# QwenLM/Qwen3-TTS

Measured on AMD Instinct MI355X. Metric: speech-tokens/sec (+ audio RTF), Qwen3-TTS-12Hz-1.7B batch=8, higher is better.
Workload: dtype bf16; 1 GPU; Qwen3-TTS-12Hz-1.7b dims, seeded random weights, batch=8 per GPU, ragged prompts 36..64 rows, 125 frames (10.0 s) per utterance, sampling T=0.9 top-k=50 rep=1.05; prefill + AR decode (hipGraph=on) + codec decode to 24 kHz (bf16); global_batch=8, frames_per_utterance=125, parallelism=request-shard x1

## Files before the change

qwen3-tts_amd/csrc/gemm_tap.hip:

```cpp
#include <map>
#include <mutex>
#include <type_traits>
#include "common.h"
#include "kernels.h"
#include "tstamp.h"

QTTS_TS_UNIT(tap)

namespace qtts {

typedef __bf16 hw_bf16x2 __attribute__((ext_vector_type(2)));
__device__ __forceinline__ unsigned cvt_pk_bf16(float a, float b) {
    hw_bf16x2 v = {(__bf16)a, (__bf16)b};
    return *reinterpret_cast<unsigned*>(&v);
}

template <bool FAST>
__device__ __forceinline__ float snake1(float v, float ea, float ib) {
    float sn;
    if constexpr (FAST) sn = __builtin_amdgcn_sinf(v * ea * 0.15915494309189535f); else sn = sinf(v * ea);
    return v + ib * (sn * sn);
}

template <int BN, int TM, int TN, bool FAST>
// ... 618 lines not shown
        gd_dma_wait();
        __syncthreads();
        if (s + 1 < nsteps) {
            const int ks2 = (s + 1) / p.taps, tap2 = (s + 1) - ks2 * p.taps;
            dma_w(ks2, tap2, (s + 1) & 1);
            if (ks2 != ks) dma_a(ks2, ks2 & 1);
        }
        const bf16_t* Ab = reinterpret_cast<const bf16_t*>(Abuf + (ks & 1) * a_stride);
        const bf16_t* Wb = reinterpret_cast<const bf16_t*>(Wbuf + (s & 1) * W_BYTES);
        const int sh = p.shift[tap];
#pragma unroll
        for (int kk = 0; kk < BK / 32; ++kk) {
            bf16x8 a[TM], b[TN];
#pragma unroll
            for (int i = 0; i < TM; ++i) {
                a[i] = *reinterpret_cast<const bf16x8*>(&Ab[(wm * 64 + i * 16 + li + halo + sh) * STR + kk * 32 + lq * 8]);
                if (tpos[i] + sh < 0) a[i] = (bf16x8){0, 0, 0, 0, 0, 0, 0, 0};
            }
#pragma unroll
            for (int j = 0; j < TN; ++j)
                b[j] = *reinterpret_cast<const bf16x8*>(&Wb[(wn * (BN / 2) + j * 16 + li) * STR + kk * 32 + lq * 8]);
#pragma unroll
            for (int i = 0; i < TM; ++i)
#pragma unroll
                for (int j = 0; j < TN; ++j)
                    acc[i][j] = __builtin_amdgcn_mfma_f32_16x16x32_bf16(b[j], a[i], acc[i][j], 0, 0, 0);
        }
    }
    tap_epilogue<BN, TM, TN, true>(p, acc, m0, n0, wm, wn, li, lq);
}

template <int BN>
static void launch_dma(const GemmTapParams& p, int halo, hipStream_t st) {
    const int nb = cdiv(p.M, 128) * cdiv(p.N, BN);
    const int a_stride = ((128 + halo) * 144 + 1023) / 1024 * 1024;
    const size_t lds = 2 * (size_t)a_stride + 2 * (size_t)((BN * 144 + 1023) / 1024 * 1024);
    auto kern = gemm_dma_kernel<BN>;
    ensure_dynamic_lds(reinterpret_cast<const void*>(kern), 160 * 1024);
    hipLaunchKernelGGL(kern, dim3(nb), dim3(256), lds, st, p, halo, a_stride);
}

__device__ __forceinline__ void ring_wait_vm(int n) {
#ifndef QTTS_HOST_EMU
    switch (n) {
        case 0: asm volatile("s_waitcnt vmcnt(0)" ::: "memory"); break;
        case 2: asm volatile("s_waitcnt vmcnt(2)" ::: "memory"); break;
        case 4: asm volatile("s_waitcnt vmcnt(4)" ::: "memory"); break;
        case 6: asm volatile("s_waitcnt vmcnt(6)" ::: "memory"); break;
        case 8: asm volatile("s_waitcnt vmcnt(8)" ::: "memory"); break;
        case 10: asm volatile("s_waitcnt vmcnt(10)" ::: "memory"); break;
        case 12: asm volatile("s_waitcnt vmcnt(12)" ::: "memory"); break;
        case 14: asm volatile("s_waitcnt vmcnt(14)" ::: "memory"); break;
        case 16: asm volatile("s_waitcnt vmcnt(16)" ::: "memory"); break;
        case 20: asm volatile("s_waitcnt vmcnt(20)" ::: "memory"); break;
        case 24: asm volatile("s_waitcnt vmcnt(24)" ::: "memory"); break;
        case 28: asm volatile("s_waitcnt vmcnt(28)" ::: "memory"); break;
        default: asm volatile("s_waitcnt vmcnt(0)" ::: "memory"); break;
    }
#else
    (void)n;
#endif
}
__device__ __forceinline__ void ring_barrier() {
#ifndef QTTS_HOST_EMU
    asm volatile("s_waitcnt lgkmcnt(0)" ::: "memory");
    __builtin_amdgcn_s_barrier();
    __builtin_amdgcn_sched_barrier(0);
#else
    __syncthreads();
#endif
}
#ifndef QTTS_RING_SGB_ALT
#define QTTS_RING_SGB_ALT 0
#endif
#define QTTS_RING_SGB (QTTS_RING_SGB_ALT == 0 ? 3 : (QTTS_RING_SGB_ALT == 1 ? 0 : QTTS_RING_SGB_ALT))
__device__ __forceinline__ void ring_sched_fence() {
#ifndef QTTS_HOST_EMU
    __builtin_amdgcn_sched_barrier(0);
#endif
}
template <int N> __device__ __forceinline__ void ring_wait_vm_c() {
#ifndef QTTS_HOST_EMU
    asm volatile("s_waitcnt vmcnt(%0)" ::"n"(N) : "memory");
#endif
}
template <int NST, int AH, bool RING_A, int TAPS = 0, int ABL = 0>
__global__ __launch_bounds__(256, 2) void gemm_ring_kernel(GemmTapParams p, int halo, int nbands ,
                                                                 int ks , f32x4* ks_ws, unsigned* ks_cnt) {
    constexpr int BM = 128, BN = 128, TM = 4, TN = 4;
    constexpr int WT = 8192;
    constexpr int D = NST;
    constexpr int LPS = RING_A ? 4 : 2;
    static_assert(!RING_A || AH == 1, "a plain Linear runs 32-wide slabs");
    extern __shared__ __attribute__((aligned(16))) unsigned char smem_gr[];
    unsigned char* Wbuf = smem_gr;
    unsigned char* Abuf = smem_gr + NST * WT;

    const int tid = threadIdx.x;
    const int lane = tid & 63;
    const int wave = __builtin_amdgcn_readfirstlane(tid >> 6);
    const int wm = wave >> 1, wn = wave & 1;
    const int li = lane & 15, lq = lane >> 4;
    const int n_tiles_n = (p.N + BN - 1) / BN;
    const int nblk = gridDim.x;
    int bid = blockIdx.x;
    {
// ... 394 lines not shown
    tab[{dev, st}] = w;
    return w;
}
static int ring_splits(const GemmTapParams& p, int nst, int ah, int n_cu) {
    const int tiles = cdiv(p.M, 128) * cdiv(p.N, 128);
    const int slabs = p.K / (32 * ah), steps = slabs * p.taps * ah;
    int ks = QTTS_OPT_INT("QTTS_GEMM_RING_KS", 0);
    (void)n_cu;
    if (ks == 0) ks = 1;
    while (ks > 1 && (slabs % ks != 0 || tiles * ks > RING_KS_MAX_PARTS || steps / ks < 2 * nst || p.act == ACT_SWIGLU)) --ks;
    return ks < 1 ? 1 : ks;
}
template <int NST, int AH, bool RING_A, int TAPS = 0, int ABL = 0>
static void launch_ring_t(const GemmTapParams& p, int halo, hipStream_t st) {
    static const int n_cu = [] {
        int dev = 0, n = 0;
        if (hipGetDevice(&dev) != hipSuccess || hipDeviceGetAttribute(&n, hipDeviceAttributeMultiprocessorCount, dev) != hipSuccess || n <= 0) n = 256;
        return n;
    }();
    const int nb = cdiv(p.M, 128) * cdiv(p.N, 128);
    const int nbands = (128 + halo + 15) / 16;
    int ks = ring_splits(p, NST, AH, n_cu);
    RingKsWs w{};
    if (ks > 1) { w = ring_ks_ws(st); if (!w.ws) ks = 1; }
    auto kern = gemm_ring_kernel<NST, AH, RING_A, TAPS, ABL>;
    ensure_dynamic_lds(reinterpret_cast<const void*>(kern), 160 * 1024);
    hipLaunchKernelGGL(kern, dim3(nb * ks), dim3(256), (size_t)ring_lds_bytes(NST, AH, p.taps, halo), st, p, halo, nbands, ks, w.ws, w.cnt);
}
static void launch_ring(const GemmTapParams& p, int halo, hipStream_t st) {
    QTTS_REQUIRE((size_t)p.M * p.lda * 2 < (1ull << 32) && (size_t)p.taps * p.N * p.K * 2 < (1ull << 32), QTTS_ERR_LIMIT, "gemm_ring: an operand of 4 GiB or more");
    int nst = QTTS_OPT_INT("QTTS_GEMM_RING_NST", 0);
    if (nst != 4 && nst != 6 && nst != 8) nst = 4;
    const int unroll = QTTS_OPT_INT("QTTS_GEMM_RING_UNROLL", 1);
    if (p.taps == 1) { if (nst == 8) launch_ring_t<8, 1, true>(p, halo, st); else launch_ring_t<4, 1, true>(p, halo, st); return; }
    while (nst > p.taps * 2) nst -= 2;
    QTTS_REQUIRE(nst >= 4, QTTS_ERR_ARG, "gemm_ring: ring deeper than a slab");
#if defined(QTTS_ABLATE) && !defined(QTTS_HOST_EMU)
    if (const int abl = QTTS_OPT_INT("QTTS_GEMM_RING_ABLATE", 0); abl && p.taps == 7) {
        switch (abl) {
            case 1: launch_ring_t<4, 2, false, 7, 1>(p, halo, st); return;
            case 2: launch_ring_t<4, 2, false, 7, 2>(p, halo, st); return;
            case 3: launch_ring_t<4, 2, false, 7, 3>(p, halo, st); return;
            case 4: launch_ring_t<4, 2, false, 7, 4>(p, halo, st); return;
            case 8: launch_ring_t<4, 2, false, 7, 8>(p, halo, st); return;
            case 7: launch_ring_t<4, 2, false, 7, 7>(p, halo, st); return;
            case 15: launch_ring_t<4, 2, false, 7, 15>(p, halo, st); return;
            default: break;
        }
    }
#endif
    if (unroll && p.taps == 7) { if (nst == 8) launch_ring_t<8, 2, false, 7>(p, halo, st); else launch_ring_t<4, 2, false, 7>(p, halo, st); return; }
    if (unroll && p.taps == 2) { launch_ring_t<4, 2, false, 2>(p, halo, st); return; }
    if (nst == 8) launch_ring_t<8, 2, false>(p, halo, st); else if (nst == 6) launch_ring_t<6, 2, false>(p, halo, st); else launch_ring_t<4, 2, false>(p, halo, st);
}

template <int BM, int BN, bool A16, int BK>
static void launch_wide_k(const GemmTapParams& p, hipStream_t st) {
    const int nb = cdiv(p.M, BM) * cdiv(p.N, BN);
    const size_t lds = (size_t)(BM + BN) * (BK + 8) * 2;
    auto kern = gemm_wide_kernel<BM, BN, A16, BK>;
    ensure_dynamic_lds(reinterpret_cast<const void*>(kern), 160 * 1024);
    hipLaunchKernelGGL(kern, dim3(nb), dim3(256), lds, st, p);
}
struct WideTile { int bm, bn, bk; };
static int g_wide_force = -1;
static WideTile wide_tile(const GemmTapParams& p, bool a16, int bn_max) {
    const int force_env = QTTS_OPT_INT("QTTS_GEMM_WIDE_TILE", 0);
    const int force = g_wide_force >= 0 ? g_wide_force : force_env;
    WideTile best{128, bn_max, 128};
    static const int n_cu = [] {
        int dev = 0, n = 0;
        if (hipGetDevice(&dev) != hipSuccess || hipDeviceGetAttribute(&n, hipDeviceAttributeMultiprocessorCount, dev) != hipSuccess || n <= 0) n = 256;
        return n;
    }();
    double tb = 1e30;
    const double ab = a16 ? 2.0 : 4.0;
    for (int cm : {128, 64, 32})
        for (int cn : {128, 64, 32})
            for (int ck : {128, 256}) {
                if (cn > bn_max || p.N % cn != 0 || p.K % ck != 0) continue;
                if (cm == 32 && (p.M > 128 || ck != 256 || cn > 64)) continue;
                if (cn == 32 && (cm != 32 || p.act == ACT_SWIGLU)) continue;
                if (ck == 256 && cm == 64 && !a16 && cn != 64) continue;
                if (ck == 256 && cm == 128) continue;
                if (force && force != (cm * 1000 + cn) * 1000 + ck) continue;
                const int wgs = cdiv(p.M, cm) * cdiv(p.N, cn), steps = p.K / ck;
                const double sb = ck * (cm * ab + cn * 2.0) * 1e-3;
                const double chain = steps * (0.53 + sb / 65.0);
                const double cu = cdiv(wgs, n_cu) * steps * sb / 80.0;
                const double op = (double)cdiv(p.M, cm) * p.N * p.K * 2.0 / 6e6;
                const double t = std::max(chain, std::max(cu, op)) * (1.0 + 0.01 * (cm * cn < 128 * 128));
                if (t < tb) { tb = t; best = {cm, cn, ck}; }
            }
    return best;
}
template <bool A16>
static void launch_wide(const GemmTapParams& p, int bn_max, hipStream_t st) {
    const WideTile t = wide_tile(p, A16, bn_max);
    if (t.bm == 32) { if (t.bn == 64) launch_wide_k<32, 64, A16, 256>(p, st); else launch_wide_k<32, 32, A16, 256>(p, st); return; }
    if (t.bm == 128) { if (t.bn == 128) launch_wide_k<128, 128, A16, 128>(p, st); else launch_wide_k<128, 64, A16, 128>(p, st); }
    else if (t.bk == 128) { if (t.bn == 128) launch_wide_k<64, 128, A16, 128>(p, st); else launch_wide_k<64, 64, A16, 128>(p, st); }
    else if (t.bn == 128) { if constexpr (A16) launch_wide_k<64, 128, true, 256>(p, st); else launch_wide_k<64, 128, false, 128>(p, st); }
    else launch_wide_k<64, 64, A16, 256>(p, st);
}

template <int BN, bool BF16>
static void launch_t(const GemmTapParams& p, hipStream_t st) {
    const int nb = cdiv(p.M, 128) * cdiv(p.N, BN);
    hipLaunchKernelGGL((gemm_tap_kernel<BN, BF16>), dim3(nb), dim3(256), 0, st, p);
}

void launch_gemm_tap(const GemmTapParams& p_in, bool bf16, hipStream_t st) {
    GemmTapParams p = p_in;
    const int wide_max_tiles = [] { const char* e = QTTS_ENV("QTTS_GEMM_WIDE_MAX"); return e && atoi(e) > 0 ? atoi(e) : 2048; }();
    QTTS_REQUIRE(p.K % 32 == 0, QTTS_ERR_ARG, "gemm_tap: K must be a multiple of 32");
    QTTS_REQUIRE(p.taps >= 1 && p.taps <= 8, QTTS_ERR_ARG, "gemm_tap: 1..8 taps");
    QTTS_REQUIRE(p.M > 0 && p.N > 0, QTTS_ERR_ARG, "gemm_tap: empty problem");
    QTTS_REQUIRE(p.lda % 4 == 0, QTTS_ERR_ARG, "gemm_tap: lda must be a multiple of 4");
    auto al16 = [](const void* q) { return reinterpret_cast<uintptr_t>(q) % 16 == 0; };
    p.vec4 = p.N % 4 == 0 && p.ldc % 4 == 0 && (!p.res || p.ldr % 4 == 0) && (!p.C16 || (p.ldc16 % 4 == 0 && reinterpret_cast<uintptr_t>(p.C16) % 8 == 0)) &&
             (!p.res16 || (p.ldres16 % 4 == 0 && reinterpret_cast<uintptr_t>(p.res16) % 8 == 0)) &&
             (!p.R16 || (p.ldR16 % 4 == 0 && reinterpret_cast<uintptr_t>(p.R16) % 8 == 0)) &&
             al16(p.C) && al16(p.res) && al16(p.bias) && al16(p.scale) && al16(p.snake_ea) && al16(p.snake_ib) && al16(p.snake16_ea) &&
             al16(p.snake16_ib) && (p.snake16_period % 4 == 0);
    if (p.act == ACT_SWIGLU) QTTS_REQUIRE(p.ldc % 4 == 0 && al16(p.C) && (!p.C16 || (p.ldc16 % 4 == 0 && reinterpret_cast<uintptr_t>(p.C16) % 8 == 0)),
                                          QTTS_ERR_ARG, "gemm_tap: swiglu outputs must be 16-byte (fp32) / 8-byte (bf16) aligned with ldc % 4 == 0");
    if (p.A16 && bf16 && p.taps == 1 && p.shift[0] == 0 && p.K % 128 == 0 && p.K >= 512 && p.N % 64 == 0 && p.lda % 8 == 0 && (p.C || p.C16) && !p.res16 &&
        !p.R16 && (cdiv(p.M, 128) * cdiv(p.N, 128) <= wide_max_tiles || p.act == ACT_SWIGLU)) {
        if (p.act == ACT_SWIGLU) QTTS_REQUIRE(p.N % 32 == 0, QTTS_ERR_ARG, "gemm_tap: swiglu needs N % 32 == 0");
        {
            const int dma_env2 = [] { const char* e = QTTS_ENV("QTTS_GEMM_DMA"); return e ? atoi(e) : 0; }();
            const int ring_env = QTTS_OPT_INT("QTTS_GEMM_RING", 1);
            if (dma_env2 == 0 && (ring_env == 2 || (ring_env == 1 && cdiv(p.M, 128) * (p.N / 128) >= 128)) && p.N % 128 == 0 && p.K % 64 == 0) {
                launch_ring(p, 0, st);
                QTTS_CHECK_HIP(hipGetLastError());
                return;
            }
            if ((dma_env2 == 1 || dma_env2 == 2) && p.N % 128 == 0 && p.K % 64 == 0 && cdiv(p.M, 128) * (p.N / 128) >= 128) {
                launch_dma<128>(p, 0, st);
                QTTS_CHECK_HIP(hipGetLastError());
                return;
            }
        }
        launch_wide<true>(p, p.N % 128 == 0 ? 128 : 64, st);
        QTTS_CHECK_HIP(hipGetLastError());
        return;
    }
    if (p.A16) {
        QTTS_REQUIRE(bf16, QTTS_ERR_ARG, "gemm_tap: A16 needs bf16 weights");
        QTTS_REQUIRE(p.act != ACT_SWIGLU, QTTS_ERR_ARG, "gemm_tap: the A16 kernel has no SwiGLU epilogue");
        QTTS_REQUIRE(p.lda % 8 == 0, QTTS_ERR_ARG, "gemm_tap: bf16 A needs lda % 8 == 0");
        QTTS_REQUIRE(p.C || p.C16 || p.R16, QTTS_ERR_ARG, "gemm_tap: no output");
        QTTS_REQUIRE(!(p.res && p.res16), QTTS_ERR_ARG, "gemm_tap: residual given twice");
        int halo = 0;
        for (int i = 0; i < p.taps; ++i) { QTTS_REQUIRE(p.shift[i] <= 0, QTTS_ERR_ARG, "gemm_tap: shift > 0"); halo = std::max(halo, -p.shift[i]); }
        QTTS_REQUIRE(halo <= 56, QTTS_ERR_LIMIT, "gemm_tap: tap reach > 56 rows");
        const int bn2 = (p.N % 128 == 0) ? 128 : (p.N % 96 == 0 ? 96 : (p.N <= 64 ? 64 : 128));
        const int bk_env = QTTS_OPT_INT("QTTS_TAP2_BK", 0);
        static const int n_cu2 = [] {
            int dev = 0, n = 0;
            if (hipGetDevice(&dev) != hipSuccess || hipDeviceGetAttribute(&n, hipDeviceAttributeMultiprocessorCount, dev) != hipSuccess || n <= 0) n = 256;
            return n;
        }();
        const int dma_env = [] { const char* e = QTTS_ENV("QTTS_GEMM_DMA"); return e ? atoi(e) : -1; }();
        const int ring_env = QTTS_OPT_INT("QTTS_GEMM_RING", 1);
        if (dma_env != 0 && bn2 == 128 && p.K % 64 == 0 && (ring_env == 2 || (ring_env == 1 && p.taps > 1))) { launch_ring(p, halo, st); QTTS_CHECK_HIP(hipGetLastError()); return; }
        if (dma_env != 0 && bn2 == 128 && p.K % 64 == 0) { launch_dma<128>(p, halo, st); QTTS_CHECK_HIP(hipGetLastError()); return; }
        const int tiles = cdiv(p.M, 128) * cdiv(p.N, bn2);
        const bool bk64 = p.K % 64 == 0 && bn2 == 128 && (bk_env == 64 || (bk_env == 0 && tiles <= n_cu2));
        if (bk64) launch_tap2<128, 64>(p, halo, st);
        else if (bn2 == 128) launch_tap2<128, 32>(p, halo, st); else if (bn2 == 96) launch_tap2<96, 32>(p, halo, st); else launch_tap2<64, 32>(p, halo, st);
        QTTS_CHECK_HIP(hipGetLastError());
        return;
    }
    QTTS_REQUIRE(p.C || (p.C16 && p.act == ACT_SWIGLU), QTTS_ERR_ARG, "gemm_tap: null output");
    QTTS_REQUIRE(!p.res16 && !p.R16, QTTS_ERR_ARG, "gemm_tap: the bf16 residual stream needs the A16 kernel");
    int bn;
    if (p.act == ACT_SWIGLU) {
        QTTS_REQUIRE(p.N % 32 == 0, QTTS_ERR_ARG, "gemm_tap: swiglu needs N % 32 == 0");
        bn = (p.N % 128 == 0) ? 128 : 64;
    } else if (p.N % 128 == 0) bn = 128;
    else if (p.N % 96 == 0) bn = 96;
    else if (p.N <= 64) bn = 64;
    else bn = 128;
    if (bf16 && p.taps == 1 && p.shift[0] == 0 && p.K % 128 == 0 && p.K >= 512 && (bn == 128 || bn == 64) &&
        cdiv(p.M, 128) * cdiv(p.N, bn) <= wide_max_tiles) {
        launch_wide<false>(p, bn, st);
        QTTS_CHECK_HIP(hipGetLastError());
        return;
    }
    if (bf16) {
        if (bn == 128) launch_t<128, true>(p, st);
        else if (bn == 96) launch_t<96, true>(p, st);
        else launch_t<64, true>(p, st);
    } else {
        if (bn == 128) launch_t<128, false>(p, st);
        else if (bn == 96) launch_t<96, false>(p, st);
        else launch_t<64, false>(p, st);
    }
    QTTS_CHECK_HIP(hipGetLastError());
}

extern "C" __attribute__((visibility("default"))) void qtts_debug_gemm_wide_tile(int32_t code) { g_wide_force = code; }
extern "C" __attribute__((visibility("default")))
void qtts_debug_gemm_wide_choice(int32_t M, int32_t N, int32_t K, int32_t a16, int32_t* bm, int32_t* bn, int32_t* bk) {
    GemmTapParams p{};
    p.M = M; p.N = N; p.K = K; p.taps = 1;
    const WideTile t = wide_tile(p, a16 != 0, N % 128 == 0 ? 128 : 64);
    *bm = t.bm; *bn = t.bn; *bk = t.bk;
}

extern "C" __attribute__((visibility("default")))
int qtts_debug_gemm_tap(int32_t M, int32_t N, int32_t K, int32_t act, int32_t with_res, int32_t a16, int32_t iters, int32_t reps,
                        double* us_per_launch) {
    try {
        QTTS_REQUIRE(us_per_launch && iters > 0 && reps > 0 && M > 0, QTTS_ERR_ARG, "bad argument");
        DevBuf A, W, Cb, R;
        A.alloc((size_t)M * K * 4); W.alloc((size_t)N * K * 2); Cb.alloc((size_t)M * N * 4); R.alloc((size_t)M * N * 4);
        QTTS_CHECK_HIP(hipMemset(A.p, 0x3c, A.bytes)); QTTS_CHECK_HIP(hipMemset(W.p, 0x3c, W.bytes)); QTTS_CHECK_HIP(hipMemset(R.p, 0, R.bytes));
        GemmTapParams p{};
        if (a16) p.A16 = A.p; else p.A = A.as<float>();
        p.lda = K; p.M = M; p.T = M; p.W = W.p; p.N = N; p.K = K; p.taps = 1; p.act = act;
        const int No = act == ACT_SWIGLU ? N / 2 : N;
        if (with_res) { p.res = R.as<float>(); p.ldr = No; }
        p.C = Cb.as<float>(); p.ldc = No;
        hipStream_t st;
        QTTS_CHECK_HIP(hipStreamCreateWithFlags(&st, hipStreamNonBlocking));
        launch_gemm_tap(p, true, st);
        QTTS_CHECK_HIP(hipStreamSynchronize(st));
        hipGraph_t gr; hipGraphExec_t ge;
        QTTS_CHECK_HIP(hipStreamBeginCapture(st, hipStreamCaptureModeThreadLocal));
        for (int i = 0; i < iters; ++i) launch_gemm_tap(p, true, st);
        QTTS_CHECK_HIP(hipStreamEndCapture(st, &gr));
        QTTS_CHECK_HIP(hipGraphInstantiate(&ge, gr, nullptr, nullptr, 0));
        QTTS_CHECK_HIP(hipGraphLaunch(ge, st)); QTTS_CHECK_HIP(hipStreamSynchronize(st));
        hipEvent_t a, b;
        QTTS_CHECK_HIP(hipEventCreate(&a)); QTTS_CHECK_HIP(hipEventCreate(&b));
        float best = 1e30f;
        for (int r = 0; r < reps; ++r) {
            QTTS_CHECK_HIP(hipEventRecord(a, st)); QTTS_CHECK_HIP(hipGraphLaunch(ge, st)); QTTS_CHECK_HIP(hipEventRecord(b, st));
            QTTS_CHECK_HIP(hipStreamSynchronize(st));
            float ms = 0; QTTS_CHECK_HIP(hipEventElapsedTime(&ms, a, b)); best = std::min(best, ms);
        }
        *us_per_launch = 1000.0 * best / iters;
        (void)hipEventDestroy(a); (void)hipEventDestroy(b); (void)hipGraphExecDestroy(ge); (void)hipGraphDestroy(gr); (void)hipStreamDestroy(st);
        return QTTS_OK;
    } catch (const qtts::Error& e) { qtts::set_last_error(e.what()); return e.code; }
    catch (const std::exception& e) { qtts::set_last_error(e.what()); return QTTS_ERR_ARG; }
}

extern "C" __attribute__((visibility("default")))
int qtts_debug_gemm_tap16(const void* A16_host, int32_t lda, int32_t M, int32_t T, const void* W_host, int32_t N, int32_t K, int32_t taps,
                          const int32_t* shift, float* C_host, int32_t iters, int32_t reps, double* us_per_launch) {
    try {
        QTTS_REQUIRE(A16_host && W_host && shift && M > 0 && T > 0 && N > 0 && K > 0 && taps >= 1 && taps <= 8 && lda >= K, QTTS_ERR_ARG, "bad argument");
        DevBuf A, W, Cb;
        A.alloc((size_t)M * lda * 2); W.alloc((size_t)taps * N * K * 2); Cb.alloc((size_t)M * N * 4);
        QTTS_CHECK_HIP(hipMemcpy(A.p, A16_host, A.bytes, hipMemcpyHostToDevice));
        QTTS_CHECK_HIP(hipMemcpy(W.p, W_host, W.bytes, hipMemcpyHostToDevice));
        QTTS_CHECK_HIP(hipMemset(Cb.p, 0xff, Cb.bytes));
        GemmTapParams p{};
        p.A16 = A.p; p.lda = lda; p.M = M; p.T = T; p.W = W.p; p.N = N; p.K = K; p.taps = taps;
// ... 33 lines not shown
```

qwen3-tts_amd/csrc/talker_engine.hip:

```cpp
#include <atomic>
#include <map>
#include <mutex>
#include <algorithm>
#include "common.h"
#include "kernels.h"
#include "glue.h"


using namespace qtts;

namespace {

struct LayerW {
    int fs_o = 16, fs_d = 16;
    DevBuf qkv_p, o_p, gu_p, d_p;
    DevBuf gu_p8;
    DevBuf o_p16;
    DevBuf gu_mlp, d_p16;
    DevBuf qkv_r, o_r, gu_r, d_r;
    bool w8 = false;
    DevBuf qkv_s, o_s, gu_s, gu8_s, d_s;
    DevBuf g1, g2, qn, kn;
};
struct StackDims { int H, I, nh, nkv, hd, qd, kvd; float eps; };
// ... 925 lines not shown
        p.res = res; p.ldr = H;
        if (out16) { p.C16 = C; p.ldc16 = ldc; p.ldc = ldc; } else { p.C = C; p.ldc = ldc; }
        launch_gemm_tap(p, bf16, st);
    };
    for (int l = 0; l < c.num_hidden_layers; ++l) {
        auto& L = tl[l];
        if (a16) launch_rmsnorm16(xs, H, L.g1.as<float>(), td.eps, nb, H, M, H, st);
        else launch_rmsnorm(xs, H, L.g1.as<float>(), td.eps, nb, H, M, H, st);
        gemm(L.qkv_r, W, H, nb, H, qb, W, ACT_NONE, nullptr);
        QkNormRopeParams q{};
        q.qkv = qb; q.ld = W; q.B = nB; q.T = T; q.nh = td.nh; q.nkv = td.nkv; q.hd = td.hd; q.qw = L.qn.as<float>();
        q.kw = L.kn.as<float>(); q.eps = td.eps; q.inv_freq = inv_freq_t.as<float>(); q.n_pad = npad_dev;
        q.kv = kv_t; q.layer = l; q.row_map = row_map; q.slot_base = slot_base;
        launch_qknorm_rope_store(q, st);
        AttnRowsParams a{};
        a.qkv = qb; a.ld = W; a.q_off = 0; a.k_off = td.qd; a.v_off = td.qd + td.kvd; a.B = nB; a.T = T; a.nh = td.nh;
        a.nkv = td.nkv; a.hd = td.hd; a.window = 0; a.n_pad = npad_dev; a.out = ab; a.ldo = td.qd;
        if (a16) a.out16 = ab;
        launch_attn_rows(a, st);
        gemm(L.o_r, H, td.qd, ab, td.qd, xs, H, ACT_NONE, xs);
        if (a16) launch_rmsnorm16(xs, H, L.g2.as<float>(), td.eps, nb, H, M, H, st);
        else launch_rmsnorm(xs, H, L.g2.as<float>(), td.eps, nb, H, M, H, st);
        gemm(L.gu_r, 2 * td.I, H, nb, H, mb, td.I, ACT_SWIGLU, nullptr, a16);
        gemm(L.d_r, H, td.I, mb, td.I, xs, H, ACT_NONE, xs);
    }
}

void qtts_talker::prefill(const float* embeds, int B_, int T, const int32_t* n_pad_host, const float* trailing_dev,
                          int Tt_, const float* tts_pad_dev, hipStream_t st) {
    const auto& c = cfg;
    QTTS_REQUIRE(finalized, QTTS_ERR_STATE, "talker: finalize() first");
    QTTS_REQUIRE(B_ >= 1 && B_ <= c.max_batch, QTTS_ERR_LIMIT, "talker: batch exceeds max_batch");
    QTTS_REQUIRE(T >= 1 && T < c.max_seq, QTTS_ERR_LIMIT, "talker: prompt longer than max_seq");
    QTTS_REQUIRE(Tt_ >= 1, QTTS_ERR_ARG, "talker: trailing_text_hidden must have >= 1 row");
    for (int b = 0; b < B_; ++b) QTTS_REQUIRE(n_pad_host[b] >= 0 && n_pad_host[b] < T, QTTS_ERR_ARG, "talker: n_pad out of range");
    if (pooled()) {
        const int want = cdiv(T, 16);
        if (B_ * want > pool_pages)
            throw Error(QTTS_ERR_LIMIT, "talker: the prompts need " + std::to_string(B_ * want) + " KV pages, the pool has " + std::to_string(pool_pages));
        for (int b = 0; b < c.max_batch; ++b) pool_release(b);
        for (int b = 0; b < B_; ++b) pool_grant(b, want);
        pool_flush(st);
    }
    B = B_; T0 = T; Tt = Tt_;
    const int M = B * T, H = td.H;
    pf_x.ensure((size_t)M * H * 4);
    trailing.ensure((size_t)B * Tt * H * 4); tts_pad.ensure((size_t)H * 4);
    QTTS_CHECK_HIP(hipMemcpyAsync(pf_x.p, embeds, (size_t)M * H * 4, hipMemcpyDeviceToDevice, st));
    QTTS_CHECK_HIP(hipMemcpyAsync(trailing.p, trailing_dev, (size_t)B * Tt * H * 4, hipMemcpyDeviceToDevice, st));
    QTTS_CHECK_HIP(hipMemcpyAsync(tts_pad.p, tts_pad_dev, (size_t)H * 4, hipMemcpyDeviceToDevice, st));
    QTTS_CHECK_HIP(hipMemcpyAsync(n_pad_d.p, n_pad_host, (size_t)B * 4, hipMemcpyHostToDevice, st));
    prefill_stack(B, T, n_pad_d.as<int>(), nullptr, 0, st);
    float* xs = pf_x.as<float>();
    for (int b = 0; b < B; ++b)
        QTTS_CHECK_HIP(hipMemcpyAsync(x.as<float>() + (size_t)b * H, xs + ((size_t)b * T + T - 1) * H, (size_t)H * 4,
                                      hipMemcpyDeviceToDevice, st));
    launch_rmsnorm(x.as<float>(), H, t_norm.as<float>(), td.eps, past_hidden.as<float>(), H, B, H, st);
    int init[6] = {0, -1, T - 1, 0, 0, 0};
    QTTS_CHECK_HIP(hipMemcpyAsync(ss.n_generated, init, sizeof(init), hipMemcpyHostToDevice, st));
    std::vector<int> ones(B, 1);
    QTTS_CHECK_HIP(hipMemcpyAsync(ss.unfinished, ones.data(), (size_t)B * 4, hipMemcpyHostToDevice, st));
    SkinnyParams h{};
    h.x = past_hidden.as<float>(); h.ldx = H; h.M = B; h.Wp = head_p.p; h.N = c.vocab_size; h.K = H;
    h.out = logits.as<float>(); h.ldo = c.vocab_size; h.act = ACT_NONE; h.fs = fs_head;
    launch_skinny(h, bf16, st);
    QTTS_CHECK_HIP(hipStreamSynchronize(st));
    prefilled = true;
}

void qtts_talker::sample_talker(const qtts_sampling& sp, int eos, int min_new, int max_new, hipStream_t st) {
    SampleParams p{};
    p.logits = logits.as<float>(); p.ld = cfg.vocab_size; p.V = cfg.vocab_size; p.B = B;
    p.generated = generated.as<int>(); p.gen_stride = gen_cap; p.n_generated_dev = ss.n_generated;
    p.repetition_penalty = sp.repetition_penalty; p.eos = eos; p.min_new_tokens = min_new;
    p.suppress_mask = suppress.as<unsigned char>();
    p.do_sample = sp.do_sample; p.top_k = sp.top_k; p.top_p = sp.top_p; p.temperature = sp.temperature;
    p.seed = sp.seed; p.seed_dev = seed_d.as<unsigned long long>(); p.stream_id = 0; p.step_dev = ss.n_generated;
    p.tok_out = cur_tok.as<int>(); p.tok_stride = 1; p.unfinished = ss.unfinished; p.generated_out = generated.as<int>();
    p.max_new_tokens = max_new; p.done_in = ss.done;
    if (row_mode) { p.rows = rows_d.as<SampleRow>(); p.rows_sub = 0; p.rows_fast = row_fast_t; }
    if (tf.codes && tf.trace) launch_teacher(teacher_params(), 0, st);
    if (row_mode && row_warp_t) { SampleWarpParams pw{p, warp_d.as<RowWarpers>(), proc_d.as<RowProcessors>()}; launch_sample_warp(pw, st); }
    else launch_sample(p, st);
    launch_sample_finish(ss, B, max_new, st);
    if (tf.codes) launch_teacher(teacher_params(), 1, st);
}

void qtts_talker::frame_step(const qtts_sampling& sp, int eos, int min_new, int max_new, int64_t* codes, float* hidden,
                             int max_frames, hipStream_t st) {
    const auto& c = cfg;
    const int G = c.num_code_groups;
    const int64_t fused_before = cp_attn_o_count, mlp_before = cp_mlp_count, layer_before = cp_layer_count, ks_before = ks_split_count, gq_before = attn_gq_count;
    cur_stack = 1;
    for (int j = 0; j < G - 1; ++j) {
        const int n_new = j == 0 ? 2 : 1, M = n_new * B;
        CpGatherParams gp{};
        gp.pass = j; gp.B = B; gp.H = td.H; gp.past_hidden = past_hidden.as<float>(); gp.talker_emb = emb_talker.as<float>();
        gp.cur_tok = cur_tok.as<int>(); gp.cp_emb = emb_cp.as<float>(); gp.cp_vocab = c.cp_vocab_size;
        gp.sub = sub.as<int>(); gp.sub_stride = G; gp.done = ss.done;
        unsigned short* c16 = bf16 ? cp_x16.as<unsigned short>() : nullptr;
        if (has_proj && j >= 1) {
        } else
        if (has_proj) {
            gp.out = cp_in.as<float>(); gp.out16 = bf16 ? cp_in16.as<unsigned short>() : nullptr;
            if (!skinny_only && j == 0) launch_cp_gather(gp, st);
            SkinnyParams pj{};
            pj.done_flag = ss.done;
            pj.x = cp_in.as<float>(); pj.ldx = td.H; pj.M = M; pj.Wp = proj_p.p; pj.N = cd.H; pj.K = td.H;
            if (bf16) { pj.x = reinterpret_cast<const float*>(cp_in16.as<unsigned short>()); pj.x_bf16 = 1; }
            pj.bias = proj_b.as<float>(); pj.out = cp_x.as<float>(); pj.ldo = cd.H; pj.act = ACT_NONE; pj.fs = fs_proj;
// ... 1047 lines not shown
    if (tokens_dev) {
        const int B = t->B, cap = g.admitting ? g.max_row : g.max_new;
        std::vector<int> h((size_t)B * cap);
        copy_on_stream(h.data(), t->generated.p, h.size() * 4, hipMemcpyDeviceToHost, st);
        std::vector<int64_t> w(h.size(), -1);
        for (int b = 0; b < B; ++b)
            for (int i = 0; i < n_tok - (g.admitting ? g.tab[b].origin : 0) && i < cap; ++i) w[(size_t)b * cap + i] = h[(size_t)b * cap + i];
        copy_on_stream(tokens_dev, w.data(), w.size() * 8, hipMemcpyHostToDevice, st);
    }
    QTTS_API_END
}

int qtts_talker_debug_logits(qtts_talker* t, float* logits_dev, void* stream) {
    QTTS_API_BEGIN
    QTTS_REQUIRE(t && logits_dev, QTTS_ERR_ARG, "null argument");
    QTTS_CHECK_HIP(hipMemcpyAsync(logits_dev, t->logits.p, (size_t)t->B * t->cfg.vocab_size * 4, hipMemcpyDeviceToDevice,
                                  (hipStream_t)stream));
    QTTS_API_END
}
int qtts_talker_debug_kv_table(qtts_talker* t, int32_t row, int32_t* entries_host, void* stream) {
    QTTS_API_BEGIN
    QTTS_REQUIRE(t && entries_host, QTTS_ERR_ARG, "null argument");
    QTTS_REQUIRE(t->finalized, QTTS_ERR_STATE, "debug_kv_table before finalize");
    QTTS_REQUIRE(row >= 0 && row < t->cfg.max_batch, QTTS_ERR_ARG, "debug_kv_table: row " + std::to_string(row) + " is not a row of this engine");
    const int pps = t->kv_t.pages_per_seq;
    copy_on_stream(entries_host, t->ptab_t.as<int>() + (size_t)row * pps, (size_t)pps * 4, hipMemcpyDeviceToHost, (hipStream_t)stream);
    QTTS_API_END
}
int qtts_talker_debug_cp_logits(qtts_talker* t, float* logits_dev, void* stream) {
    QTTS_API_BEGIN
    QTTS_REQUIRE(t && logits_dev, QTTS_ERR_ARG, "null argument");
    const size_t Vc = (size_t)t->cfg.cp_vocab_size;
    for (int j = 0; j < t->cfg.num_code_groups - 1; ++j)
        QTTS_CHECK_HIP(hipMemcpyAsync(logits_dev + (size_t)j * t->B * Vc, t->cp_logits.as<float>() + (size_t)j * 64 * Vc, (size_t)t->B * Vc * 4,
                                      hipMemcpyDeviceToDevice, (hipStream_t)stream));
    QTTS_API_END
}
__global__ void xcc_probe_kernel(int* out) {
#ifndef QTTS_HOST_EMU
    if (threadIdx.x == 0) out[blockIdx.x] = (int)__builtin_amdgcn_s_getreg((31 << 11) | 20) & 0xf;
#else
    if (threadIdx.x == 0) out[blockIdx.x] = blockIdx.x & 7;
#endif
}
int qtts_debug_xcc_map(int32_t grid, int32_t* out_host, void* stream) {
    QTTS_API_BEGIN
    QTTS_REQUIRE(grid >= 1 && grid <= 65536 && out_host, QTTS_ERR_ARG, "xcc_map: grid 1..65536");
    DevBuf d; d.alloc((size_t)grid * 4);
    hipLaunchKernelGGL(xcc_probe_kernel, dim3(grid), dim3(256), 0, (hipStream_t)stream, d.as<int>());
    QTTS_CHECK_HIP(hipStreamSynchronize((hipStream_t)stream));
    QTTS_CHECK_HIP(hipMemcpy(out_host, d.p, (size_t)grid * 4, hipMemcpyDeviceToHost));
    QTTS_API_END
}
int qtts_debug_cp_layer_occupancy(int32_t H, int32_t I, int32_t bf16) {
    try { return qtts::cp_layer_blocks_per_cu(H, I, bf16 != 0); } catch (...) { return -1; }
}
int qtts_talker_get_stats(qtts_talker* t, qtts_talker_stats* out) {
    QTTS_API_BEGIN
    QTTS_REQUIRE(t && out, QTTS_ERR_ARG, "null argument");
    out->frames_run = t->frames_run; out->graph_nodes = t->graph_nodes; out->weight_bytes_per_frame = t->weight_bytes_frame;
    out->gemm_ms_last = t->prof_ms; out->gemm_launches_last = t->prof_launches;
    out->long_graphs = (int32_t)t->graph_long.size(); out->attn_nsplit_last = t->attn_nsplit_active; out->attn_span_last = t->attn_span_active;
    out->cp_fused_per_step = t->cp_fused_slot ? t->cp_fused_per_step : 0;
    out->cp_fused_launches_last = (int64_t)out->cp_fused_per_step * t->frames_run;
    out->cp_fused_giveups = t->cp_fused_giveups; out->cp_fused_capacity = t->fused_capacity; out->cp_fused_active = t->cp_fused_slot ? 1 : 0;
    out->cp_mlp_per_step = t->cp_fused_slot ? t->cp_mlp_per_step : 0;
    out->cp_layer_per_step = t->cp_fused_slot ? t->cp_layer_per_step : 0;
    out->ks_split_per_step = t->ks_split_env ? t->ks_split_per_step : 0; out->attn_gq_per_step = t->attn_gq_per_step;
    out->graph_captures = t->graph_captures; out->row_table_last = t->row_mode ? 1 : 0;
    out->admit_calls = (int32_t)t->admit_calls; out->admitted_rows = (int32_t)t->admitted_rows;
    QTTS_API_END
}
int qtts_talker_get_gemm_profile(qtts_talker* t, qtts_gemm_class* out, int32_t cap, int32_t* n) {
    QTTS_API_BEGIN
    QTTS_REQUIRE(t && n && (out || cap == 0), QTTS_ERR_ARG, "null argument");
    *n = (int32_t)t->prof_classes.size();
    for (int i = 0; i < *n && i < cap; ++i) out[i] = t->prof_classes[i];
    QTTS_API_END
}
__global__ void null_kernel(int* p, int mode) {
    if (mode == 1) { if (*p) return; }
    if (mode == 2) { __shared__ int s[64]; s[threadIdx.x & 63] = threadIdx.x; __syncthreads(); if (threadIdx.x == 0 && s[5] == 12345) *p = 1; }
}
int qtts_debug_null_chain(int32_t grid, int32_t block, int32_t mode, int32_t iters, int32_t reps, double* us) {
    QTTS_API_BEGIN
    DevBuf d; d.alloc(64); QTTS_CHECK_HIP(hipMemset(d.p, 0, 64));
    hipStream_t st; QTTS_CHECK_HIP(hipStreamCreateWithFlags(&st, hipStreamNonBlocking));
    hipGraph_t gr; hipGraphExec_t ge;
    QTTS_CHECK_HIP(hipStreamBeginCapture(st, hipStreamCaptureModeThreadLocal));
    for (int i = 0; i < iters; ++i) hipLaunchKernelGGL(null_kernel, dim3(grid), dim3(block), 0, st, d.as<int>(), mode);
    QTTS_CHECK_HIP(hipStreamEndCapture(st, &gr));
    QTTS_CHECK_HIP(hipGraphInstantiate(&ge, gr, nullptr, nullptr, 0));
    QTTS_CHECK_HIP(hipGraphLaunch(ge, st)); QTTS_CHECK_HIP(hipStreamSynchronize(st));
    hipEvent_t a, b; QTTS_CHECK_HIP(hipEventCreate(&a)); QTTS_CHECK_HIP(hipEventCreate(&b));
    float best = 1e30f;
    for (int r = 0; r < reps; ++r) {
        QTTS_CHECK_HIP(hipEventRecord(a, st)); QTTS_CHECK_HIP(hipGraphLaunch(ge, st)); QTTS_CHECK_HIP(hipEventRecord(b, st));
        QTTS_CHECK_HIP(hipStreamSynchronize(st));
        float ms = 0; QTTS_CHECK_HIP(hipEventElapsedTime(&ms, a, b)); best = std::min(best, ms);
    }
    *us = 1000.0 * best / iters;
    (void)hipEventDestroy(a); (void)hipEventDestroy(b); (void)hipGraphExecDestroy(ge); (void)hipGraphDestroy(gr); (void)hipStreamDestroy(st);
    QTTS_API_END
}

int qtts_debug_skinny_chain(int32_t N, int32_t K, int32_t M, int32_t act, int32_t with_norm, int32_t with_res,
// ... 79 lines not shown
```

Baseline: 48310 speech-tokens/s.

## Add smaller-tile DMA ring GEMM for mid-size prefill linears; fuse last-row gather

Adds a new ring-buffered direct-to-LDS GEMM kernel with 64x64 or 128x64 tiles. A planner selects it for prefill-sized linears (M 129..2048, large N and K) whose 128x128 tile count would not fill the CUs, so the grid covers more compute units. Separately, the per-batch device-to-device copies of the last prefill row are removed by having rmsnorm read strided rows directly. It also adds debug entry points, and the new kernel adds more code paths and relies on hand-tuned waitcnt scheduling.

```diff
diff --git a/qwen3-tts_amd/csrc/gemm_tap.hip b/qwen3-tts_amd/csrc/gemm_tap.hip
--- a/qwen3-tts_amd/csrc/gemm_tap.hip
+++ b/qwen3-tts_amd/csrc/gemm_tap.hip
@@ -694,6 +694,7 @@
         case 12: asm volatile("s_waitcnt vmcnt(12)" ::: "memory"); break;
         case 14: asm volatile("s_waitcnt vmcnt(14)" ::: "memory"); break;
         case 16: asm volatile("s_waitcnt vmcnt(16)" ::: "memory"); break;
+        case 18: asm volatile("s_waitcnt vmcnt(18)" ::: "memory"); break;
         case 20: asm volatile("s_waitcnt vmcnt(20)" ::: "memory"); break;
         case 24: asm volatile("s_waitcnt vmcnt(24)" ::: "memory"); break;
         case 28: asm volatile("s_waitcnt vmcnt(28)" ::: "memory"); break;
@@ -1194,6 +1195,176 @@
     if (unroll && p.taps == 7) { if (nst == 8) launch_ring_t<8, 2, false, 7>(p, halo, st); else launch_ring_t<4, 2, false, 7>(p, halo, st); return; }
     if (unroll && p.taps == 2) { launch_ring_t<4, 2, false, 2>(p, halo, st); return; }
     if (nst == 8) launch_ring_t<8, 2, false>(p, halo, st); else if (nst == 6) launch_ring_t<6, 2, false>(p, halo, st); else launch_ring_t<4, 2, false>(p, halo, st);
+}
+
+template <int BM, int BN, int KS, int NST>
+__global__ __launch_bounds__(256, 2) void gemm_ring_kernel_m(GemmTapParams p) {
+    constexpr int TM = BM / 32, TN = BN / 32;
+    constexpr int AQ = BM / 64, WQ = BN / 64;
+    constexpr int SUB = (BM + BN) * 64;
+    constexpr int ST = KS * SUB;
+    constexpr int LPS = KS * (AQ + WQ);
+    constexpr int D = NST;
+    static_assert(BM % 64 == 0 && BN % 64 == 0 && NST >= 3, "whole bands per wave; a ring of at least three stages");
+    extern __shared__ __attribute__((aligned(16))) unsigned char smem_gr[];
+
+    const int tid = threadIdx.x;
+    const int lane = tid & 63;
+    const int wave = __builtin_amdgcn_readfirstlane(tid >> 6);
+    const int wm = wave >> 1, wn = wave & 1;
+    const int li = lane & 15, lq = lane >> 4;
+    const int n_tiles_n = (p.N + BN - 1) / BN;
+    const int nblk = gridDim.x;
+    int bid = blockIdx.x;
+    {
+        const int q = nblk / 8, r = nblk % 8, xcd = bid % 8, idx = bid / 8;
+        bid = (xcd < r ? xcd * (q + 1) : r * (q + 1) + (xcd - r) * q) + idx;
+    }
+    const int m0 = (bid / n_tiles_n) * BM;
+    const int n0 = (bid % n_tiles_n) * BN;
+    const unsigned char* A16 = reinterpret_cast<const unsigned char*>(p.A16);
+    const unsigned char* Wg = reinterpret_cast<const unsigned char*>(p.W);
+
+    const int d_row = lane >> 2, d_chunk = (lane & 3) ^ ((lane >> 3) & 2);
+    unsigned a_off[AQ], w_off[WQ];
+#pragma unroll
+    for (int i = 0; i < AQ; ++i) {
+        int gr = m0 + (wave + 4 * i) * 16 + d_row;
+        gr = gr < p.M ? gr : p.M - 1;
+        a_off[i] = ((unsigned)gr * (unsigned)p.lda + d_chunk * 8) * 2u;
+    }
+#pragma unroll
+    for (int i = 0; i < WQ; ++i) {
+        int gn = n0 + (wave + 4 * i) * 16 + d_row;
+        gn = gn < p.N ? gn : p.N - 1;
+        w_off[i] = ((unsigned)gn * (unsigned)p.K + d_chunk * 8) * 2u;
+    }
+    const int nsteps = p.K / (32 * KS);
+    int rt = 0, r_stage = 0;
+    unsigned r_k = 0;
+    auto request_next = [&]() {
+        unsigned char* dst = smem_gr + r_stage * ST;
+#pragma unroll
+        for (int h = 0; h < KS; ++h) {
+#pragma unroll
+            for (int i = 0; i < AQ; ++i) gd_dma16(A16 + (a_off[i] + r_k + h * 64u), dst + h * SUB + (wave + 4 * i) * 1024);
+#pragma unroll
+            for (int i = 0; i < WQ; ++i) gd_dma16(Wg + (w_off[i] + r_k + h * 64u), dst + h * SUB + BM * 64 + (wave + 4 * i) * 1024);
+        }
+        ++rt;
+        r_stage = r_stage + 1 == NST ? 0 : r_stage + 1;
+        r_k += KS * 64u;
+    };
+
+    f32x4 acc[TM][TN];
+#pragma unroll
+    for (int i = 0; i < TM; ++i)
+#pragma unroll
+        for (int j = 0; j < TN; ++j) acc[i][j] = (f32x4){0.f, 0.f, 0.f, 0.f};
+    const int sw = (lq ^ ((li >> 1) & 2)) << 4;
+    const int afrag = (wm * (BM / 2) + li) * 64 + sw;
+    const int wfrag = BM * 64 + (wn * (BN / 2) + li) * 64 + sw;
+    int f_stage = 0;
+    auto read_frags = [&](bf16x8 (&a)[KS][TM], bf16x8 (&b)[KS][TN]) {
+        const unsigned char* src = smem_gr + f_stage * ST;
+#pragma unroll
+        for (int h = 0; h < KS; ++h) {
+#pragma unroll
+            for (int i = 0; i < TM; ++i) a[h][i] = *reinterpret_cast<const bf16x8*>(src + h * SUB + afrag + i * 1024);
+#pragma unroll
+            for (int j = 0; j < TN; ++j) b[h][j] = *reinterpret_cast<const bf16x8*>(src + h * SUB + wfrag + j * 1024);
+        }
+        f_stage = f_stage + 1 == NST ? 0 : f_stage + 1;
+    };
+
+    for (int t = 0; t < D && t < nsteps; ++t) request_next();
+    {
+        const int later = (D < nsteps ? D : nsteps) - 1;
+        ring_wait_vm(LPS * later);
+        ring_barrier();
+    }
+    bf16x8 fa[2][KS][TM], fb[2][KS][TN];
+    read_frags(fa[0], fb[0]);
+    auto step = [&](auto steady, int t, bf16x8 (&ca)[KS][TM], bf16x8 (&cb)[KS][TN], bf16x8 (&na)[KS][TM], bf16x8 (&nb)[KS][TN]) {
+        constexpr bool STEADY = decltype(steady)::value;
+        if constexpr (STEADY) ring_wait_vm_c<LPS * (D - 2)>();
+        else { int later = nsteps - 2 - t; later = later < D - 2 ? later : D - 2; later = later > 0 ? later : 0; ring_wait_vm(LPS * later); }
+        ring_barrier();
+        if constexpr (STEADY) request_next();
+        else if (rt < nsteps) request_next();
+#pragma unroll
+        for (int j = 0; j < TN; ++j) acc[0][j] = __builtin_amdgcn_mfma_f32_16x16x32_bf16(cb[0][j], ca[0][0], acc[0][j], 0, 0, 0);
+        ring_sched_fence();
+        if constexpr (STEADY) read_frags(na, nb);
+        else if (t + 1 < nsteps) read_frags(na, nb);
+#pragma unroll
+        for (int h = 0; h < KS; ++h)
+#pragma unroll
+            for (int i = (h == 0 ? 1 : 0); i < TM; ++i)
+#pragma unroll
+                for (int j = 0; j < TN; ++j)
+                    acc[i][j] = __builtin_amdgcn_mfma_f32_16x16x32_bf16(cb[h][j], ca[h][i], acc[i][j], 0, 0, 0);
+#ifndef QTTS_HOST_EMU
+        if constexpr (STEADY) {
+#pragma unroll
+            for (int k = 0; k < KS * TM * TN - TN; ++k) {
+                __builtin_amdgcn_sched_group_barrier(0x008, 1, 0);
+                __builtin_amdgcn_sched_group_barrier(0x096, 3, 0);
+            }
+        }
+#endif
+        ring_sched_fence();
+    };
+    int t = 0;
+    for (; t + 1 < nsteps - D; t += 2) {
+        step(std::true_type{}, t, fa[0], fb[0], fa[1], fb[1]);
+        step(std::true_type{}, t + 1, fa[1], fb[1], fa[0], fb[0]);
+    }
+#pragma unroll 1
+    for (; t < nsteps; t += 2) {
+        step(std::false_type{}, t, fa[0], fb[0], fa[1], fb[1]);
+        if (t + 1 < nsteps) step(std::false_type{}, t + 1, fa[1], fb[1], fa[0], fb[0]);
+    }
+    tap_epilogue<BN, TM, TN, true>(p, acc, m0, n0, wm, wn, li, lq);
+}
+
+constexpr int RING_M_CODE = 1000000000;
+static bool ring_m_admits(const GemmTapParams& p, int bm, int bn, int kstep) {
+    return p.A16 && p.taps == 1 && p.shift[0] == 0 && p.K % kstep == 0 && p.K / kstep >= 2 && p.N % 64 == 0 && p.lda % 8 == 0 && !p.res16 && !p.R16 &&
+           (size_t)p.M * p.lda * 2 < (1ull << 32) && (size_t)p.N * p.K * 2 < (1ull << 32) && (p.act != ACT_SWIGLU || p.N % 32 == 0) && bm > 0 && bn > 0;
+}
+template <int BM, int BN, int KS, int NST>
+static void launch_ring_m_t(const GemmTapParams& p, hipStream_t st) {
+    const int nb = cdiv(p.M, BM) * cdiv(p.N, BN);
+    auto kern = gemm_ring_kernel_m<BM, BN, KS, NST>;
+    ensure_dynamic_lds(reinterpret_cast<const void*>(kern), 160 * 1024);
+    hipLaunchKernelGGL(kern, dim3(nb), dim3(256), (size_t)NST * KS * (BM + BN) * 64, st, p);
+}
+static bool ring_m_code_admits(const GemmTapParams& p, int code) {
+    const int t = code - RING_M_CODE, bm = t / 1000000, bn = t / 1000 % 1000, kstep = t % 1000;
+    return (t == 64064064 || t == 128064064) && ring_m_admits(p, bm, bn, kstep);
+}
+static bool launch_ring_m(const GemmTapParams& p, int code, hipStream_t st) {
+    if (!ring_m_code_admits(p, code)) return false;
+    switch (code - RING_M_CODE) {
+        case 64064064: launch_ring_m_t<64, 64, 2, 4>(p, st); return true;
+        case 128064064: launch_ring_m_t<128, 64, 2, 4>(p, st); return true;
+        default: return false;
+    }
+}
+static int prefill_lin_tile(const GemmTapParams& p) {
+    static const int n_cu = [] {
+        int dev = 0, n = 0;
+        if (hipGetDevice(&dev) != hipSuccess || hipDeviceGetAttribute(&n, hipDeviceAttributeMultiprocessorCount, dev) != hipSuccess || n <= 0) n = 256;
+        return n;
+    }();
+    const int env = QTTS_OPT_INT("QTTS_GEMM_RING_M", 1);
+    if (env == 0 || p.M < 129 || p.M > 2048) return 0;
+    if (env >= RING_M_CODE) return env;
+    if (p.N < 2048 || p.K < 2048 || p.N % 128 != 0 || cdiv(p.M, 128) * (p.N / 128) >= n_cu) return 0;
+    if (cdiv(p.M, 64) * (p.N / 64) <= n_cu) return RING_M_CODE + 64064064;
+    if (cdiv(p.M, 128) * (p.N / 64) <= n_cu) return RING_M_CODE + 128064064;
+    return 0;
 }
 
 template <int BM, int BN, bool A16, int BK>
@@ -1252,6 +1423,20 @@
     hipLaunchKernelGGL((gemm_tap_kernel<BN, BF16>), dim3(nb), dim3(256), 0, st, p);
 }
 
+enum { LIN_WIDE = 0, LIN_RING = 1, LIN_DMA = 2, LIN_RING_M = 3 };
+struct LinPlan { int kind, code; };
+static LinPlan plan_lin16(const GemmTapParams& p) {
+    const int dma_env2 = [] { const char* e = QTTS_ENV("QTTS_GEMM_DMA"); return e ? atoi(e) : 0; }();
+    const int ring_env = QTTS_OPT_INT("QTTS_GEMM_RING", 1);
+    const int force = g_wide_force >= 0 ? g_wide_force : QTTS_OPT_INT("QTTS_GEMM_WIDE_TILE", 0);
+    const int rl = force >= RING_M_CODE ? force : (force == 0 && dma_env2 == 0 && ring_env == 1 ? prefill_lin_tile(p) : 0);
+    if (rl && ring_m_code_admits(p, rl)) return {LIN_RING_M, rl};
+    const bool big = cdiv(p.M, 128) * (p.N / 128) >= 128 && p.N % 128 == 0 && p.K % 64 == 0;
+    if (force == 0 && dma_env2 == 0 && p.N % 128 == 0 && p.K % 64 == 0 && (ring_env == 2 || (ring_env == 1 && big))) return {LIN_RING, 0};
+    if (force == 0 && (dma_env2 == 1 || dma_env2 == 2) && big) return {LIN_DMA, 0};
+    return {LIN_WIDE, 0};
+}
+
 void launch_gemm_tap(const GemmTapParams& p_in, bool bf16, hipStream_t st) {
     GemmTapParams p = p_in;
     const int wide_max_tiles = [] { const char* e = QTTS_ENV("QTTS_GEMM_WIDE_MAX"); return e && atoi(e) > 0 ? atoi(e) : 2048; }();
@@ -1270,20 +1455,10 @@
     if (p.A16 && bf16 && p.taps == 1 && p.shift[0] == 0 && p.K % 128 == 0 && p.K >= 512 && p.N % 64 == 0 && p.lda % 8 == 0 && (p.C || p.C16) && !p.res16 &&
         !p.R16 && (cdiv(p.M, 128) * cdiv(p.N, 128) <= wide_max_tiles || p.act == ACT_SWIGLU)) {
         if (p.act == ACT_SWIGLU) QTTS_REQUIRE(p.N % 32 == 0, QTTS_ERR_ARG, "gemm_tap: swiglu needs N % 32 == 0");
-        {
-            const int dma_env2 = [] { const char* e = QTTS_ENV("QTTS_GEMM_DMA"); return e ? atoi(e) : 0; }();
-            const int ring_env = QTTS_OPT_INT("QTTS_GEMM_RING", 1);
-            if (dma_env2 == 0 && (ring_env == 2 || (ring_env == 1 && cdiv(p.M, 128) * (p.N / 128) >= 128)) && p.N % 128 == 0 && p.K % 64 == 0) {
-                launch_ring(p, 0, st);
-                QTTS_CHECK_HIP(hipGetLastError());
-                return;
-            }
-            if ((dma_env2 == 1 || dma_env2 == 2) && p.N % 128 == 0 && p.K % 64 == 0 && cdiv(p.M, 128) * (p.N / 128) >= 128) {
-                launch_dma<128>(p, 0, st);
-                QTTS_CHECK_HIP(hipGetLastError());
-                return;
-            }
-        }
+        const LinPlan pl = plan_lin16(p);
+        if (pl.kind == LIN_RING_M && launch_ring_m(p, pl.code, st)) { QTTS_CHECK_HIP(hipGetLastError()); return; }
+        if (pl.kind == LIN_RING) { launch_ring(p, 0, st); QTTS_CHECK_HIP(hipGetLastError()); return; }
+        if (pl.kind == LIN_DMA) { launch_dma<128>(p, 0, st); QTTS_CHECK_HIP(hipGetLastError()); return; }
         launch_wide<true>(p, p.N % 128 == 0 ? 128 : 64, st);
         QTTS_CHECK_HIP(hipGetLastError());
         return;
@@ -1350,6 +1525,49 @@
     p.M = M; p.N = N; p.K = K; p.taps = 1;
     const WideTile t = wide_tile(p, a16 != 0, N % 128 == 0 ? 128 : 64);
     *bm = t.bm; *bn = t.bn; *bk = t.bk;
+}
+
+extern "C" __attribute__((visibility("default")))
+void qtts_debug_gemm_lin_plan(int32_t M, int32_t N, int32_t K, int32_t act, int32_t* kind, int32_t* bm, int32_t* bn, int32_t* bk) {
+    GemmTapParams p{};
+    p.A16 = &p; p.lda = K; p.M = M; p.N = N; p.K = K; p.taps = 1; p.act = act;
+    const LinPlan pl = plan_lin16(p);
+    *kind = pl.kind;
+    if (pl.kind == LIN_RING_M) { const int t = pl.code - RING_M_CODE; *bm = t / 1000000; *bn = t / 1000 % 1000; *bk = t % 1000; }
+    else if (pl.kind == LIN_WIDE) { const WideTile t = wide_tile(p, true, N % 128 == 0 ? 128 : 64); *bm = t.bm; *bn = t.bn; *bk = t.bk; }
+    else { *bm = 128; *bn = 128; *bk = pl.kind == LIN_RING ? 32 : 64; }
+}
+
+extern "C" __attribute__((visibility("default")))
+int qtts_debug_gemm_lin16(const void* A16_host, int32_t M, const void* W_host, int32_t N, int32_t K, int32_t act, const float* res_host,
+                          float* C_host, void* C16_host) {
+    try {
+        QTTS_REQUIRE(A16_host && W_host && M > 0 && N > 0 && K > 0 && (C_host || C16_host) && (act == ACT_NONE || act == ACT_SWIGLU), QTTS_ERR_ARG, "bad argument");
+        const int No = act == ACT_SWIGLU ? N / 2 : N;
+        DevBuf A, W, Cb, Ch, R;
+        A.alloc((size_t)M * K * 2); W.alloc((size_t)N * K * 2); Cb.alloc((size_t)M * No * 4); Ch.alloc((size_t)M * No * 2);
+        QTTS_CHECK_HIP(hipMemcpy(A.p, A16_host, A.bytes, hipMemcpyHostToDevice));
+        QTTS_CHECK_HIP(hipMemcpy(W.p, W_host, W.bytes, hipMemcpyHostToDevice));
+        QTTS_CHECK_HIP(hipMemset(Cb.p, 0xff, Cb.bytes)); QTTS_CHECK_HIP(hipMemset(Ch.p, 0xff, Ch.bytes));
+        GemmTapParams p{};
+        p.A16 = A.p; p.lda = K; p.M = M; p.T = M; p.W = W.p; p.N = N; p.K = K; p.taps = 1; p.act = act;
+        if (res_host) {
+            R.alloc((size_t)M * No * 4);
+            QTTS_CHECK_HIP(hipMemcpy(R.p, res_host, R.bytes, hipMemcpyHostToDevice));
+            p.res = R.as<float>(); p.ldr = No;
+        }
+        if (C_host) { p.C = Cb.as<float>(); p.ldc = No; }
+        if (C16_host) { p.C16 = Ch.p; p.ldc16 = No; }
+        hipStream_t st;
+        QTTS_CHECK_HIP(hipStreamCreateWithFlags(&st, hipStreamNonBlocking));
+        launch_gemm_tap(p, true, st);
+        QTTS_CHECK_HIP(hipStreamSynchronize(st));
+        if (C_host) QTTS_CHECK_HIP(hipMemcpy(C_host, Cb.p, Cb.bytes, hipMemcpyDeviceToHost));
+        if (C16_host) QTTS_CHECK_HIP(hipMemcpy(C16_host, Ch.p, Ch.bytes, hipMemcpyDeviceToHost));
+        (void)hipStreamDestroy(st);
+        return QTTS_OK;
+    } catch (const qtts::Error& e) { qtts::set_last_error(e.what()); return e.code; }
+    catch (const std::exception& e) { qtts::set_last_error(e.what()); return QTTS_ERR_ARG; }
 }
 
 extern "C" __attribute__((visibility("default")))
diff --git a/qwen3-tts_amd/csrc/talker_engine.hip b/qwen3-tts_amd/csrc/talker_engine.hip
--- a/qwen3-tts_amd/csrc/talker_engine.hip
+++ b/qwen3-tts_amd/csrc/talker_engine.hip
@@ -1001,10 +1001,7 @@
     QTTS_CHECK_HIP(hipMemcpyAsync(n_pad_d.p, n_pad_host, (size_t)B * 4, hipMemcpyHostToDevice, st));
     prefill_stack(B, T, n_pad_d.as<int>(), nullptr, 0, st);
     float* xs = pf_x.as<float>();
-    for (int b = 0; b < B; ++b)
-        QTTS_CHECK_HIP(hipMemcpyAsync(x.as<float>() + (size_t)b * H, xs + ((size_t)b * T + T - 1) * H, (size_t)H * 4,
-                                      hipMemcpyDeviceToDevice, st));
-    launch_rmsnorm(x.as<float>(), H, t_norm.as<float>(), td.eps, past_hidden.as<float>(), H, B, H, st);
+    launch_rmsnorm(xs + (size_t)(T - 1) * H, T * H, t_norm.as<float>(), td.eps, past_hidden.as<float>(), H, B, H, st);
     int init[6] = {0, -1, T - 1, 0, 0, 0};
     QTTS_CHECK_HIP(hipMemcpyAsync(ss.n_generated, init, sizeof(init), hipMemcpyHostToDevice, st));
     std::vector<int> ones(B, 1);
@@ -2158,6 +2155,19 @@
     QTTS_CHECK_HIP(hipMemcpy(out_host, d.p, (size_t)grid * 4, hipMemcpyDeviceToHost));
     QTTS_API_END
 }
+int qtts_debug_talker_kv(qtts_talker* t, void* k_host, void* v_host, int64_t cap, int64_t* bytes, void* stream) {
+    QTTS_API_BEGIN
+    QTTS_REQUIRE(t && bytes, QTTS_ERR_ARG, "null argument");
+    QTTS_REQUIRE(t->finalized, QTTS_ERR_STATE, "debug_talker_kv before finalize");
+    *bytes = (int64_t)t->kpool_t.bytes;
+    if (k_host && v_host) {
+        QTTS_REQUIRE(cap >= *bytes, QTTS_ERR_ARG, "debug_talker_kv: host buffers smaller than a pool");
+        QTTS_CHECK_HIP(hipStreamSynchronize((hipStream_t)stream));
+        QTTS_CHECK_HIP(hipMemcpy(k_host, t->kpool_t.p, t->kpool_t.bytes, hipMemcpyDeviceToHost));
+        QTTS_CHECK_HIP(hipMemcpy(v_host, t->vpool_t.p, t->vpool_t.bytes, hipMemcpyDeviceToHost));
+    }
+    QTTS_API_END
+}
 int qtts_debug_cp_layer_occupancy(int32_t H, int32_t I, int32_t bf16) {
     try { return qtts::cp_layer_blocks_per_cu(H, I, bf16 != 0); } catch (...) { return -1; }
 }
```

New measurement: 48430 speech-tokens/s, median of 3. Within noise of the previous version (+0.3%).
